# ElesionKyrie/Extreme-Video-Compression-With-Prediction-Using-Pre-trainded-Diffusion-Models-

Measured on AMD Instinct MI355X. Metric: decoded frames/sec (128x128x30) at q3, higher is better.
Workload: dtype f32

## Files before the change

extreme-video-compression-with-prediction-using-pre-trainded-diffusion-models-_amd/csrc/conv_igemm.hip:

```cpp
#include <hip/hip_runtime.h>
#include <stdint.h>
#include <stdio.h>
#include "../../include/evc_hip.h"

typedef float f32x16 __attribute__((ext_vector_type(16)));
typedef __attribute__((address_space(3))) void lds_void;
typedef const __attribute__((address_space(1))) void glb_void;

#ifndef EVC_CONV_TAIL
#define EVC_CONV_TAIL 1
#endif
#ifndef EVC_CONV_TM1
#define EVC_CONV_TM1 1
#endif
#ifndef EVC_SPLIT_WIDE_TILES
#define EVC_SPLIT_WIDE_TILES 1
#endif

#ifndef EVC_SPLIT_INTERLEAVE
#define EVC_SPLIT_INTERLEAVE 5
#endif

namespace {

constexpr int BM_MAX = 128;
constexpr int KC = 16;

constexpr int MODE_PLAIN = 0, MODE_AFFINE = 1, MODE_AFFINE_SILU = 2, MODE_SILU = 3, MODE_RELU = 4;

struct ConvK {
    const float* src0; const float* src1; int C0; int C1; int ld0; int ld1;
    const float* coef_a; const float* coef_s;
    const float* w; const float* bias; const float* res; int ld_res;
    float out_scale; int act_out;
    float* out; int ld_out;
    int B, H, W, Co, CoPad, KH, KW;
    int M, HW, nchunk, nsteps, steps_per_split, splits;
    float* ws;
    float* stats;
    const float* w_hdr;
    const unsigned* in_bound;
    int tail_first, tail_splits, tail_sps, tail_rows;
    int cut_chunk;
    const float* x2_src0; const float* x2_src1; int x2_C0, x2_C1, x2_ld0, x2_ld1;
    const char* x2_w;
    const float* x2_hdr;
    const unsigned* x2_bound;
    int bound_stride, generic_epi;
};

__device__ __forceinline__ float bound_scale(unsigned bits) {
    const float b = sqrtf(__uint_as_float(bits));
    if (!(b < 3.0e38f)) return __builtin_nanf("");
    return b > 0.f ? ldexpf(1.0f, 6 - ilogbf(b)) : 1.0f;
}
__device__ __forceinline__ int bound_index(const ConvK& p, int m) { return p.bound_stride ? min(m, p.M - 1) / p.HW : 0; }
__device__ __forceinline__ float in_scale(const ConvK& p, int m) {
    if (!p.in_bound) return 1.0f;
    return bound_scale(p.in_bound[bound_index(p, m)]);
}

__device__ __forceinline__ float silu_f(float v) { return v * __builtin_amdgcn_rcpf(1.0f + __expf(-v)); }

__device__ __forceinline__ float act_fn(float v, int act) {
    if (act == EVC_ACT_SILU) return silu_f(v);
    if (act == EVC_ACT_RELU) return v < 0.f ? 0.f : v;
    return v;
}

template <int MODE>
__device__ __forceinline__ float4 transform(float4 v, const float4& a, const float4& s, bool ok) {
    if (MODE == MODE_AFFINE || MODE == MODE_AFFINE_SILU) {
        v.x = v.x * a.x + s.x; v.y = v.y * a.y + s.y; v.z = v.z * a.z + s.z; v.w = v.w * a.w + s.w;
    }
    if (MODE == MODE_AFFINE_SILU || MODE == MODE_SILU) {
        v.x = silu_f(v.x); v.y = silu_f(v.y); v.z = silu_f(v.z); v.w = silu_f(v.w);
    }
    if (MODE == MODE_RELU) {
        v.x = v.x < 0.f ? 0.f : v.x; v.y = v.y < 0.f ? 0.f : v.y; v.z = v.z < 0.f ? 0.f : v.z; v.w = v.w < 0.f ? 0.f : v.w;
    }
    v.x = ok ? v.x : 0.f; v.y = ok ? v.y : 0.f; v.z = ok ? v.z : 0.f; v.w = ok ? v.w : 0.f;
    return v;
}

template <int TM, int TN>
__device__ __forceinline__ void mfma_group(f32x16 (&acc)[TM][TN], const float4 (&a)[TM], const float4 (&b)[TN]) {
#define EVC_MFMA_E(e)                                                                                   \
    _Pragma("unroll") for (int i = 0; i < TM; ++i) _Pragma("unroll") for (int j = 0; j < TN; ++j)      \
        acc[i][j] = __builtin_amdgcn_mfma_f32_32x32x2f32(a[i].e, b[j].e, acc[i][j], 0, 0, 0);
    EVC_MFMA_E(x) EVC_MFMA_E(y) EVC_MFMA_E(z) EVC_MFMA_E(w)
#undef EVC_MFMA_E
}

template <int TM, int TN, int WM, bool PARTIAL, bool RES, bool STATS, bool ACT>
__device__ __forceinline__ void conv_epilogue_full(const ConvK& p, f32x16 (&acc)[TM][TN], int m0, int n0, int split,
                                                   int wm, int wn, int l31, int half, bool tail) {
    constexpr int BM = 32 * TM * WM;
    const int ws_m0 = tail ? p.tail_first * BM : 0;
    const size_t ws_M = tail ? (size_t)p.tail_rows : (size_t)p.M;
    const float ascale = p.w_hdr ? p.w_hdr[0] / in_scale(p, m0) : 1.0f;
// ... 966 lines not shown
            __builtin_amdgcn_sched_barrier(0);
            store_a(ab ^ 1);
            __builtin_amdgcn_sched_barrier(0);
            EVC_RR_TERMS(SP::NTERM / 2, SP::NTERM)
            __builtin_amdgcn_sched_barrier(0);
            __syncthreads();
            wb ^= 1; ++sidx;
        }
    }
#undef EVC_RR_TERMS
#undef EVC_RR_FRAGS
#undef EVC_RR_NEXT_W

    conv_epilogue<TM, TN, WM>(p, acc, m0, n0, split, wm, wn, l31, half, tail);
}

template <bool PARTIAL, bool RES, bool STATS, bool ACT>
__device__ __forceinline__ void wide_epilogue_t(const ConvK& p, f32x16 (&acc)[4][3], char* lds, int m0, int n0, int split,
                                                int wave, int lane, bool tail) {
    constexpr int TM = 4, TN = 3, BM = 256, RS = 36;
    const int wm = wave >> 1, wn = wave & 1;
    const int l31 = lane & 31, half = lane >> 5;
    const int ws_m0 = tail ? p.tail_first * BM : 0;
    const size_t ws_M = tail ? (size_t)p.tail_rows : (size_t)p.M;
    const float ascale = p.w_hdr[0] / in_scale(p, m0);
    const float oscale = p.out_scale;
    const bool has_res = RES && (!ACT || p.res != nullptr), has_stats = STATS && (!ACT || p.stats != nullptr);
    float* const patch0 = reinterpret_cast<float*>(lds) + wave * 2 * 32 * RS;
    const int wr = lane >> 3, wc = (lane & 7) * 4;
    const int mw = m0 + wm * 32 * TM;
    const int prow = 4 * half * RS + l31;
    constexpr int RD = 4;
    float4 rq[RD][4];
    const auto res_load = [&](int t, float4 (&dst)[4]) {
        const int jj = t / TM, ii = t - jj * TM;
        const float* rp = p.res + (size_t)(mw + ii * 32 + wr) * p.ld_res + n0 + wn * 32 * TN + jj * 32 + wc;
#pragma unroll
        for (int k = 0; k < 4; ++k) dst[k] = *reinterpret_cast<const float4*>(rp + (size_t)(8 * k) * p.ld_res);
    };
    if (has_res) {
#pragma unroll
        for (int t = 0; t < RD - 1; ++t) res_load(t, rq[t]);
    }
#pragma unroll
    for (int j = 0; j < TN; ++j) {
        const int cj = n0 + wn * 32 * TN + j * 32;
        const float bias = (!PARTIAL && p.bias) ? p.bias[cj + l31] : 0.f;
        float4 ssum = make_float4(0.f, 0.f, 0.f, 0.f), ssq = make_float4(0.f, 0.f, 0.f, 0.f);
#pragma unroll
        for (int i = 0; i < TM; ++i) {
            const int mb = mw + i * 32;
            const int tt = j * TM + i;
            if (has_res && tt + RD - 1 < TM * TN) res_load(tt + RD - 1, rq[(tt + RD - 1) % RD]);
            float* const P = patch0 + ((i * TN + j) & 1) * 32 * RS;
#pragma unroll
            for (int r = 0; r < 16; ++r) P[prow + ((r & 3) + 8 * (r >> 2)) * RS] = acc[i][j][r] * ascale + bias;
#pragma unroll
            for (int k = 0; k < 4; ++k) {
                float4 q = *reinterpret_cast<const float4*>(P + (wr + 8 * k) * RS + wc);
                const int m = mb + wr + 8 * k;
                if (!PARTIAL) {
                    if (has_res) { const float4& rr = rq[tt % RD][k]; q.x += rr.x; q.y += rr.y; q.z += rr.z; q.w += rr.w; }
                    q.x *= oscale; q.y *= oscale; q.z *= oscale; q.w *= oscale;
                    if (ACT) { q.x = act_fn(q.x, p.act_out); q.y = act_fn(q.y, p.act_out); q.z = act_fn(q.z, p.act_out); q.w = act_fn(q.w, p.act_out); }
                    if (STATS) {
                        ssum.x += q.x; ssum.y += q.y; ssum.z += q.z; ssum.w += q.w;
                        ssq.x += q.x * q.x; ssq.y += q.y * q.y; ssq.z += q.z * q.z; ssq.w += q.w * q.w;
                    }
                }
                float* dst = PARTIAL ? p.ws + ((size_t)split * ws_M + (m - ws_m0)) * p.Co + cj + wc
                                     : p.out + (size_t)m * p.ld_out + cj + wc;
                *reinterpret_cast<float4*>(dst) = q;
            }
            if (has_stats && (i & 1)) {
#pragma unroll
                for (int d = 8; d <= 32; d <<= 1) {
                    ssum.x += __shfl_xor(ssum.x, d); ssum.y += __shfl_xor(ssum.y, d); ssum.z += __shfl_xor(ssum.z, d); ssum.w += __shfl_xor(ssum.w, d);
                    ssq.x += __shfl_xor(ssq.x, d); ssq.y += __shfl_xor(ssq.y, d); ssq.z += __shfl_xor(ssq.z, d); ssq.w += __shfl_xor(ssq.w, d);
                }
                if (wr == 0) {
                    float* sp = p.stats + ((size_t)(m0 / 64 + wm * 2 + (i >> 1)) * p.Co + cj + wc) * 2;
                    *reinterpret_cast<float4*>(sp) = make_float4(ssum.x, ssq.x, ssum.y, ssq.y);
                    *reinterpret_cast<float4*>(sp + 4) = make_float4(ssum.z, ssq.z, ssum.w, ssq.w);
                }
                ssum = make_float4(0.f, 0.f, 0.f, 0.f); ssq = make_float4(0.f, 0.f, 0.f, 0.f);
            }
        }
    }
}

__device__ __forceinline__ void wide_epilogue(const ConvK& p, f32x16 (&acc)[4][3], char* lds, int m0, int n0, int split,
                                              int wave, int lane, bool tail) {
    const bool partial = p.splits > 1 || tail;
    if (partial) wide_epilogue_t<true, false, false, false>(p, acc, lds, m0, n0, split, wave, lane, tail);
    else if (p.act_out != EVC_ACT_NONE) wide_epilogue_t<false, true, true, true>(p, acc, lds, m0, n0, split, wave, lane, tail);
    else if (p.res && p.stats) wide_epilogue_t<false, true, true, false>(p, acc, lds, m0, n0, split, wave, lane, tail);
    else if (p.stats) wide_epilogue_t<false, false, true, false>(p, acc, lds, m0, n0, split, wave, lane, tail);
    else if (p.res) wide_epilogue_t<false, true, false, false>(p, acc, lds, m0, n0, split, wave, lane, tail);
    else wide_epilogue_t<false, false, false, false>(p, acc, lds, m0, n0, split, wave, lane, tail);
}

#ifndef EVC_WIDE_VMEM_EVERY
#define EVC_WIDE_VMEM_EVERY 36
#endif
#ifndef EVC_WIDE_BDIST
#define EVC_WIDE_BDIST 1
#endif
#ifndef EVC_WIDE_BUFFER_LOADS
#define EVC_WIDE_BUFFER_LOADS 0
#endif
#ifndef EVC_WIDE_ABL
#define EVC_WIDE_ABL 0
#endif
#ifdef EVC_WIDE_STAMPS
__device__ unsigned long long g_wide_stamps[8192 * 8];
#define EVC_STAMP(k) if (threadIdx.x == 0) g_wide_stamps[(blockIdx.x & 8191) * 8 + (k)] = __builtin_readcyclecounter();
#else
#define EVC_STAMP(k)
#endif
template <int MODE, int NU, bool X2>
__global__ __launch_bounds__(256, 1) void conv_wide_kernel(ConvK p) {
    typedef Split<2> SP;
    typedef f16x8 vec;
    constexpr int TM = 4, TN = 3, BM = 256, BN = 192, RB = 32;
    constexpr bool HAS_COEF = MODE == MODE_AFFINE || MODE == MODE_AFFINE_SILU;
    extern __shared__ __attribute__((aligned(16))) char smem_b[];
    const int W = p.W, SW = W + 2;
    const int R = BM / W;
    const int SPX = (R + 2) * SW;
    const int APL = SPX * RB;
    const int HPL = SPX * 16;
    char* const As = smem_b;

    const int tid = threadIdx.x;
    const int lane = tid & 63;
    const int wave = __builtin_amdgcn_readfirstlane(tid >> 6);
    const int wm = wave >> 1, wn = wave & 1;
    const int l31 = lane & 31, half = lane >> 5;

#ifdef EVC_WIDE_STAGGER_TEST
    if (blockIdx.x < 256) for (int q = 0; q < (int)((blockIdx.x >> 3) & 3) * EVC_WIDE_STAGGER_TEST; ++q) __builtin_amdgcn_s_sleep(127);
#endif
    EVC_STAMP(0)
    const bool tail = (int)blockIdx.x >= p.tail_first;
    const int tq = tail ? ((int)blockIdx.x - p.tail_first) / p.tail_splits : 0;
    const int m0 = (tail ? p.tail_first + tq : (int)blockIdx.x) * BM;
    const int n0 = blockIdx.y * BN;
    const int split = tail ? (int)blockIdx.x - p.tail_first - tq * p.tail_splits : (int)blockIdx.z;
    const int sps = tail ? p.tail_sps : p.steps_per_split;
    const int c_begin = p.cut_chunk ? (split ? p.cut_chunk : 0) : min(p.nchunk, split * (sps / 9));
    const int c_end = p.cut_chunk ? (split ? p.nchunk : p.cut_chunk) : min(p.nchunk, c_begin + sps / 9);

    const int bimg = m0 / p.HW;
    const int y0 = (m0 - bimg * p.HW) / W;
    const int Ct = p.C0 + p.C1;

    const int kh = tid & 1;
    unsigned goff0[NU], goff1[NU];
    int slds[NU];
    bool sval[NU], sex[NU];
#pragma unroll
    for (int k = 0; k < NU; ++k) {
        int pp = (tid + 256 * k) >> 1;
        if (pp >= (R + 2) * W) pp = tid >> 1;
        const int sr = pp / W, x = pp - sr * W;
        sex[k] = true;
        const int y = y0 + sr - 1;
        sval[k] = sex[k] && y >= 0 && y < p.H;
        const unsigned pix = (unsigned)((bimg * p.H + (sval[k] ? y : 0)) * W + x);
        goff0[k] = (pix * (unsigned)p.ld0 + 8u * kh) * 4u;
        goff1[k] = (pix * (unsigned)p.ld1 + 8u * kh) * 4u;
        const int spx = (sex[k] ? sr : 0) * SW + x + 1;
// ... 35 lines not shown
        }
    };
#endif

    const float xscale = F16_ACT_SCALE * in_scale(p, m0);
    float4 xr[NU][2], ca[2], cs[2];
    vec a[TM][2];
    auto stage_load = [&](int k, int c) {
        const int cc = c * KC;
        const bool first = cc < p.C0;
        const char* src = reinterpret_cast<const char*>(first ? p.src0 : p.src1);
        const unsigned o = (first ? goff0[k] : goff1[k]) + (unsigned)(first ? cc : cc - p.C0) * 4u;
        xr[k][0] = *reinterpret_cast<const float4*>(src + o);
        xr[k][1] = *reinterpret_cast<const float4*>(src + o + 16);
    };
    auto coef_load = [&](int c) {
        if (HAS_COEF) {
            const size_t co = (size_t)bimg * Ct + c * KC + 8 * kh;
            ca[0] = *reinterpret_cast<const float4*>(p.coef_a + co);
            ca[1] = *reinterpret_cast<const float4*>(p.coef_a + co + 4);
            cs[0] = *reinterpret_cast<const float4*>(p.coef_s + co);
            cs[1] = *reinterpret_cast<const float4*>(p.coef_s + co + 4);
        }
    };
    auto stage_store = [&](int k, int buf) {
        vec pl[2];
        SP::split(transform<MODE>(xr[k][0], ca[0], cs[0], sval[k]), transform<MODE>(xr[k][1], ca[1], cs[1], sval[k]), xscale, pl);
        char* A = As + buf * 2 * APL + slds[k];
        *reinterpret_cast<vec*>(A) = pl[0];
        *reinterpret_cast<vec*>(A + APL) = pl[1];
    };
    auto read_a = [&](int i, const char* img, int toff) {
        a[i][0] = *reinterpret_cast<const vec*>(img + abase[i] + toff);
        a[i][1] = *reinterpret_cast<const vec*>(img + APL + abase[i] + toff);
    };

    f32x16 acc[TM][TN];
#pragma unroll
    for (int i = 0; i < TM; ++i)
#pragma unroll
        for (int j = 0; j < TN; ++j)
#pragma unroll
            for (int r = 0; r < 16; ++r) acc[i][j][r] = 0.f;

    vec b[3][TN][2];
    const bool early = !X2 && c_begin < c_end;
    if (early) {
        coef_load(c_begin);
#pragma unroll
        for (int k = 0; k < NU; ++k) stage_load(k, c_begin);
        load_b(b[0], c_begin, 0);
    }
    EVC_STAMP(5)
    {
        const int nimg = X2 ? 3 : 2;
        const int per_img = (R + 2) * 2 * 4;
        for (int u = tid; u < nimg * per_img; u += 256) {
            const int img = u / per_img, q = u - img * per_img;
            const int ph = q & 3, side = (q >> 2) & 1, row = q >> 3;
            const int spx = row * SW + (side ? W + 1 : 0);
            *reinterpret_cast<float4*>(As + img * 2 * APL + (ph >> 1) * APL + (ph & 1) * HPL + spx * 16) = make_float4(0.f, 0.f, 0.f, 0.f);
        }
    }
    __syncthreads();

#define EVC_PIN(x) asm volatile("" : "+v"(x))
#define EVC_PIN4(f) asm volatile("" : "+v"((f).x), "+v"((f).y), "+v"((f).z), "+v"((f).w))
#define EVC_WIDE_MFMA_I(I, BB)                                                                          \
    _Pragma("unroll") for (int t_ = 0; t_ < SP::NTERM; ++t_)                                            \
        _Pragma("unroll") for (int j = 0; j < TN; ++j)                                                  \
            acc[I][j] = SP::mfma(a[I][SP::qa(t_)], BB[j][SP::qb(t_)], acc[I][j]);

    if constexpr (X2) {
        const int nch2 = (p.x2_C0 + p.x2_C1) / KC;
        const int nsp = tail ? p.tail_splits : p.splits;
        const int per = (nch2 + nsp - 1) / nsp;
        const int c2b = min(nch2, split * per), c2e = min(nch2, c2b + per);
        float s2 = 1.0f;
        {
            const float bb = sqrtf(__uint_as_float(p.x2_bound[bound_index(p, m0)]));
            if (!(bb < 3.0e38f)) s2 = __builtin_nanf("");
            else if (bb > 0.f) s2 = ldexpf(1.0f, 6 - ilogbf(bb));
        }
        const float xscale2 = F16_ACT_SCALE * s2;
        const unsigned slab2 = 2u * planeB;
        float4 x2r[2][2][2];
        unsigned x2o0[2], x2o1[2];
        int x2l[2];
#pragma unroll
        for (int k = 0; k < 2; ++k) {
            const int pp = (tid + 256 * k) >> 1;
            const int r = pp / W, x = pp - r * W;
            x2o0[k] = ((unsigned)(m0 + pp) * (unsigned)p.x2_ld0 + 8u * kh) * 4u;
            x2o1[k] = ((unsigned)(m0 + pp) * (unsigned)p.x2_ld1 + 8u * kh) * 4u;
            x2l[k] = kh * HPL + ((r + 1) * SW + x + 1) * 16;
        }
        auto load2 = [&](int c, float4 (&xr2)[2][2]) {
            const int cc = c * KC;
            const bool first = cc < p.x2_C0;
            const char* src = reinterpret_cast<const char*>(first ? p.x2_src0 : p.x2_src1);
            const unsigned cb = (unsigned)(first ? cc : cc - p.x2_C0) * 4u;
#pragma unroll
            for (int k = 0; k < 2; ++k) {
                const unsigned o = (first ? x2o0[k] : x2o1[k]) + cb;
                xr2[k][0] = *reinterpret_cast<const float4*>(src + o);
                xr2[k][1] = *reinterpret_cast<const float4*>(src + o + 16);
            }
        };
        auto store2 = [&](int buf, float4 (&xr2)[2][2]) {
            const float4 z = make_float4(0.f, 0.f, 0.f, 0.f);
#pragma unroll
            for (int k = 0; k < 2; ++k) {
                vec pl[2];
                SP::split(transform<MODE_PLAIN>(xr2[k][0], z, z, true), transform<MODE_PLAIN>(xr2[k][1], z, z, true), xscale2, pl);
                char* A = As + buf * 2 * APL + x2l[k];
                *reinterpret_cast<vec*>(A) = pl[0];
                *reinterpret_cast<vec*>(A + APL) = pl[1];
            }
        };
        vec b2[2][TN][2];
        auto load_b2 = [&](vec (&bb)[TN][2], int c) {
            const char* wt = p.x2_w + (unsigned)c * slab2;
#pragma unroll
            for (int j = 0; j < TN; ++j) {
                bb[j][0] = *reinterpret_cast<const vec*>(wt + wlane + j * 32 * RB);
                bb[j][1] = *reinterpret_cast<const vec*>(wt + planeB + wlane + j * 32 * RB);
            }
        };
        const int n2 = c2e - c2b;
        if (n2 > 0) {
            const auto clampc = [&](int c) { return min(c, c2e - 1); };
            load2(c2b, x2r[0]);
            load2(clampc(c2b + 1), x2r[1]);
            load_b2(b2[0], c2b);
            store2(0, x2r[0]);
            store2(1, x2r[1]);
            load2(clampc(c2b + 2), x2r[0]);
            load2(clampc(c2b + 3), x2r[1]);
            __syncthreads();
#pragma unroll
            for (int i = 0; i < TM; ++i) read_a(i, As, tap_off(4));
            int ring = 0;
#define EVC_WIDE_X2_STEP(BCUR, BNXT, XR)                                                                    \
            {                                                                                           \
                const int rn1 = ring == 2 ? 0 : ring + 1, rn2 = rn1 == 2 ? 0 : rn1 + 1;                 \
                _Pragma("unroll") for (int j = 0; j < TN; ++j) { EVC_PIN(BCUR[j][0]); EVC_PIN(BCUR[j][1]); } \
                _Pragma("unroll") for (int k = 0; k < 2; ++k) { EVC_PIN4(XR[k][0]); EVC_PIN4(XR[k][1]); } \
                load_b2(BNXT, clampc(c + 1));                                                           \
                const char* An = As + rn1 * 2 * APL;                                                    \
                _Pragma("unroll") for (int i = 0; i < TM; ++i) {                                        \
                    EVC_PIN(a[i][0]); EVC_PIN(a[i][1]);                                                 \
                    EVC_WIDE_MFMA_I(i, BCUR)                                                            \
                    read_a(i, An, tap_off(4));                                                          \
                }                                                                                       \
                store2(rn2, XR);                                                       \
                _Pragma("unroll") for (int m = 0; m < 36; ++m) {                                        \
                    if (m == 0) __builtin_amdgcn_sched_group_barrier(0x020, 6, 0);                      \
                    __builtin_amdgcn_sched_group_barrier(0x008, 1, 0);                                  \
                    __builtin_amdgcn_sched_group_barrier(0x402, 3, 0);                                  \
                    if (m % 9 == 8) __builtin_amdgcn_sched_group_barrier(0x100, 2, 0);                  \
                }                                                                                       \
                __builtin_amdgcn_sched_group_barrier(0x200, 4, 0);                                      \
                __builtin_amdgcn_sched_barrier(0);                                                      \
                load2(clampc(c + 4), XR);                                \
                asm volatile("s_waitcnt lgkmcnt(0)\n\ts_barrier" ::: "memory");                         \
                __builtin_amdgcn_sched_barrier(0);                                                      \
                ring = rn1;                                                                             \
            }
            int c = c2b;
            for (; c + 1 < c2e; c += 2) {
                EVC_WIDE_X2_STEP(b2[0], b2[1], x2r[0])
                ++c;
                EVC_WIDE_X2_STEP(b2[1], b2[0], x2r[1])
                --c;
            }
            if (c < c2e) EVC_WIDE_X2_STEP(b2[0], b2[1], x2r[0])
#undef EVC_WIDE_X2_STEP
        }
        __syncthreads();
        const float r = (p.x2_hdr[0] / s2) / (p.w_hdr[0] / in_scale(p, m0));
#pragma unroll
        for (int i = 0; i < TM; ++i)
#pragma unroll
            for (int j = 0; j < TN; ++j)
#pragma unroll
                for (int e = 0; e < 16; ++e) acc[i][j][e] *= r;
    }

    EVC_STAMP(6)
    if (c_begin < c_end) {
        if (!early) {
            coef_load(c_begin);
#pragma unroll
            for (int k = 0; k < NU; ++k) stage_load(k, c_begin);
            load_b(b[0], c_begin, 0);
        }
        if (EVC_WIDE_BDIST == 2) load_b(b[1], c_begin, 1);
#pragma unroll
        for (int k = 0; k < NU; ++k) stage_store(k, 0);
        EVC_STAMP(7)
        __syncthreads();
#pragma unroll
        for (int i = 0; i < TM; ++i) read_a(i, As, 0);
    }
    EVC_STAMP(1)
    for (int c = c_begin; c < c_end; ++c) {
        const int ab = (c - c_begin) & 1;
        const int cn = min(c + 1, c_end - 1);
        const char* Acur = As + ab * 2 * APL;
        const char* Anxt = As + (ab ^ 1) * 2 * APL;
#define EVC_WIDE_STEP(T, LOADK, STOREK, TAIL_CODE)                                                      \
        {                                                                                               \
            _Pragma("unroll") for (int j = 0; j < TN; ++j) { EVC_PIN(b[T % 3][j][0]); EVC_PIN(b[T % 3][j][1]); } \
            if constexpr (STOREK >= 0 && STOREK < NU) { EVC_PIN4(xr[STOREK < 0 ? 0 : STOREK][0]); EVC_PIN4(xr[STOREK < 0 ? 0 : STOREK][1]); } \
            if constexpr (STOREK == 0 && HAS_COEF) { EVC_PIN4(ca[0]); EVC_PIN4(ca[1]); EVC_PIN4(cs[0]); EVC_PIN4(cs[1]); } \
            if (EVC_WIDE_ABL & 64) load_b(b[(T + EVC_WIDE_BDIST) % 3], c_begin, 0);    \
            else if (!(EVC_WIDE_ABL & 2)) load_b(b[(T + EVC_WIDE_BDIST) % 3], (T + EVC_WIDE_BDIST < 9) ? c : cn, (T + EVC_WIDE_BDIST) % 9); \
            if (T == 0 && !(EVC_WIDE_ABL & 8)) coef_load(cn);                                           \
            if constexpr (LOADK >= 0 && LOADK < NU && !(EVC_WIDE_ABL & 8)) stage_load(LOADK < 0 ? 0 : LOADK, cn); \
            const char* An = (T == 8) ? Anxt : Acur;                    \
            const int toff = tap_off((T + 1) % 9);                                                      \
            _Pragma("unroll") for (int i = 0; i < TM; ++i) {                                            \
                EVC_PIN(a[i][0]); EVC_PIN(a[i][1]);                                                     \
                EVC_WIDE_MFMA_I(i, b[T % 3])                                                            \
                if (!(EVC_WIDE_ABL & 4)) read_a(i, An, toff);                                           \
            }                                                                                           \
            if constexpr (STOREK >= 0 && STOREK < NU && !(EVC_WIDE_ABL & 1)) stage_store(STOREK < 0 ? 0 : STOREK, ab ^ 1); \
             \
             \
            _Pragma("unroll") for (int m = 0; m < 36; ++m) {                                            \
                if (m % EVC_WIDE_VMEM_EVERY == 0) __builtin_amdgcn_sched_group_barrier(0x020, 1, 0);    \
                __builtin_amdgcn_sched_group_barrier(0x008, 1, 0);                                      \
                __builtin_amdgcn_sched_group_barrier(0x402, 4, 0);                                      \
                if (m % 9 == 8) __builtin_amdgcn_sched_group_barrier(0x100, 2, 0);                      \
            }                                                                                           \
            __builtin_amdgcn_sched_group_barrier(0x200, 2, 0);                                          \
            __builtin_amdgcn_sched_barrier(0);                                                          \
            TAIL_CODE                                                                                   \
            __builtin_amdgcn_sched_barrier(0);                                                          \
        }
        EVC_WIDE_STEP(0, 0, -1, )
        EVC_WIDE_STEP(1, 1, -1, )
        EVC_WIDE_STEP(2, 2, 0, )
        EVC_WIDE_STEP(3, 3, 1, )
        EVC_WIDE_STEP(4, -1, 2, )
        EVC_WIDE_STEP(5, -1, 3, )
        EVC_WIDE_STEP(6, -1, -1, )
        EVC_WIDE_STEP(7, -1, -1, asm volatile("s_waitcnt lgkmcnt(0)\n\ts_barrier" ::: "memory");)
// ... 191 lines not shown
    }
}

extern "C" int evc_conv_pack_weights(const float* w, void* packed, int Co, int Ci, int KH, int KW, int arith,
                                     void* stream) {
    if (arith == EVC_ARITH_F32) return evc_conv_pack_weights_f32(w, (float*)packed, Co, Ci, KH, KW, stream);
    if (arith != EVC_ARITH_BF16X6 && arith != EVC_ARITH_F16X3) return EVC_EINVAL;
    if (!w || !packed || Co <= 0 || Ci <= 0 || Ci % KC != 0 || KH <= 0 || KW <= 0) return EVC_EINVAL;
    const long long total = evc_conv_packed_floats(Co, Ci, KH, KW);
    int grid = (int)((total + 255) / 256 > 4096 ? 4096 : (total + 255) / 256);
    hipStream_t st = (hipStream_t)stream;
    if (arith == EVC_ARITH_BF16X6) {
        hipLaunchKernelGGL(conv_pack_split_kernel, dim3(grid), dim3(256), 0, st, w, (__bf16*)packed, Co,
                           evc_conv_co_pad(Co), Ci, KH, KW);
    } else {
        if (hipMemsetAsync(packed, 0, F16_HDR_BYTES, st) != hipSuccess) return EVC_ELAUNCH;
        const size_t n = (size_t)Co * Ci * KH * KW;
        hipLaunchKernelGGL(conv_absmax_kernel, dim3(grid), dim3(256), 0, st, w, n, reinterpret_cast<unsigned*>(packed) + 2);
        hipLaunchKernelGGL(conv_pack_f16_kernel, dim3(grid), dim3(256), 0, st, w, (char*)packed, Co,
                           evc_conv_co_pad(Co), Ci, KH, KW);
    }
    return hipGetLastError() == hipSuccess ? EVC_OK : EVC_ELAUNCH;
}

static int conv_validate(const evc_conv_args* a) {
    if (!a || !a->src0 || !a->w_packed || !a->out) return EVC_EINVAL;
    if (a->C0 <= 0 || a->C0 % KC != 0 || a->C1 < 0 || a->C1 % KC != 0) return EVC_EINVAL;
    if (a->C1 > 0 && !a->src1) return EVC_EINVAL;
    if ((a->ld0 != 0 && (a->ld0 < a->C0 || (a->ld0 & 3))) || (a->ld1 != 0 && (a->ld1 < a->C1 || (a->ld1 & 3))))
        return EVC_EINVAL;
    if ((a->coef_a == nullptr) != (a->coef_s == nullptr)) return EVC_EINVAL;
    if (a->B <= 0 || a->H <= 0 || a->W <= 0 || a->Co <= 0) return EVC_EINVAL;
    if (a->KH <= 0 || a->KW <= 0 || !(a->KH & 1) || !(a->KW & 1)) return EVC_EINVAL;
    if (a->ld_out < a->Co || (a->res && a->ld_res < a->Co)) return EVC_EINVAL;
    if ((long long)a->B * a->H * a->W > 0x7fffffffLL) return EVC_EINVAL;
    if (a->arith != EVC_ARITH_F32 && a->arith != EVC_ARITH_BF16X6 && a->arith != EVC_ARITH_F16X3) return EVC_EINVAL;
    if (a->x2_w_packed) {
        if (!a->x2_src0 || !a->x2_bound || a->x2_C0 <= 0 || a->x2_C0 % KC != 0 || a->x2_C1 < 0 || a->x2_C1 % KC != 0) return EVC_EINVAL;
        if (a->x2_C1 > 0 && !a->x2_src1) return EVC_EINVAL;
        if ((a->x2_ld0 != 0 && (a->x2_ld0 < a->x2_C0 || (a->x2_ld0 & 3))) || (a->x2_ld1 != 0 && (a->x2_ld1 < a->x2_C1 || (a->x2_ld1 & 3))))
            return EVC_EINVAL;
    }
    return EVC_OK;
}

struct TileCfg { int tm, tn, bm, bn; long long tiles; int splits; int reuse; int wide; int steps_per_split;
                 int tail_first, tail_tiles, tail_splits, tail_sps;
                 int cut_chunk; };
static int g_wide_cut = 1;
static int g_tail_split = EVC_CONV_TAIL;
static int g_wide_tiles = EVC_SPLIT_WIDE_TILES;
static int g_no_reuse = 0;
static int g_wide_mid = 1;
static int g_wide256 = 1;
static int g_force_tm = 0;

static void split_tile_cfg(const evc_conv_args* a, long long M, long long ntile, int nsteps, TileCfg& c, bool rr_ok, bool inv) {
    const double K = (double)a->KH * a->KW * (a->C0 + a->C1);
    const bool f16 = a->arith == EVC_ARITH_F16X3 && rr_ok;
    const double E = f16 ? 20.0 : 6.0, F2 = f16 ? 1.5 : 1.0;
    const auto grid_time = [&](long long n, double sps) {
        const long long R = n / 512, rem = n - R * 512;
        return (sps + E) * ((double)R * F2 + (rem == 0 ? 0.0 : (rem <= 256 && f16 ? 1.0 : F2)));
    };
    double best = 1e300;
    int best_tm = 2, best_s = 1;
    c.tail_first = 0; c.tail_tiles = 0; c.tail_splits = 1; c.tail_sps = 0;
    for (int tm = 2; tm >= 1; --tm) {
        if (!inv && g_force_tm && tm != g_force_tm) continue;
        const long long tiles = ((M + 64 * tm - 1) / (64 * tm)) * ntile;
        const int smax = a->splits > 0 ? a->splits : (nsteps / 4 < 1 ? 1 : (nsteps / 4 > 32 ? 32 : nsteps / 4));
        for (int s = a->splits > 0 ? a->splits : 1; s <= smax; ++s) {
            const double sps = (double)((nsteps + s - 1) / s);
            const double slab_mb = (double)s * (double)M * a->Co * 4.0 / 1e6;
            const double pen = s > 1 ? 1.0 + (slab_mb > 192.0 ? 300.0 : 40.0) * s / K : 1.0;
            const double tmf = tm == 1 ? (a->KH * a->KW > 1 ? 0.5 / (rr_ok ? 0.55 : 0.75) : 0.5) : 1.0;
            const double t = grid_time(tiles * s, sps) * pen * tmf;
            if (t < best * 0.9999) { best = t; best_tm = tm; best_s = s; }
        }
    }
    c.tm = best_tm;
    c.bm = 64 * c.tm;
    c.tiles = ((M + c.bm - 1) / c.bm) * ntile;
    c.splits = best_s;
    if (!inv && rr_ok && g_tail_split && a->splits <= 0 && !g_force_tm && M % 128 == 0) {
        const long long tm_all = M / 128, wgs = tm_all * ntile;
        const long long R = wgs / 512;
        const long long main_m = R * 512 / ntile, tail_m = tm_all - main_m;
        const int unit = 3 * 9;
        if (R >= 1 && tail_m > 0 && nsteps >= 2 * unit) {
            int ts = (int)(512 / (tail_m * ntile));
            if (ts > nsteps / unit) ts = nsteps / unit;
            if (ts >= 2) {
                int sps = (nsteps + ts - 1) / ts;
                sps = (sps + 2) / 3 * 3;
                ts = (nsteps + sps - 1) / sps;
                const double t_tail = grid_time(main_m * ntile, (double)nsteps) +
                                      grid_time(tail_m * ntile * ts, (double)sps) * (1.0 + 40.0 * ts / K);
                if (ts >= 2 && t_tail < best * 0.98) {
                    c.tm = 2; c.bm = 128; c.tiles = wgs; c.splits = 1;
                    c.tail_first = (int)main_m; c.tail_tiles = (int)tail_m; c.tail_splits = ts; c.tail_sps = sps;
                }
            }
        }
    }
}

static inline bool is_split_arith(int arith) { return arith == EVC_ARITH_BF16X6 || arith == EVC_ARITH_F16X3; }
static inline int arith_planes(int arith) { return arith == EVC_ARITH_F16X3 ? 2 : 3; }
constexpr long long LDS_CAP = 160 * 1024;

static long long rr_lds_bytes(int np, int bm, int W, int bn) {
    return (long long)np * 32 * (2LL * (bm / W) * (W + 2) + 2LL * bn);
}

static long long wide_lds_bytes(int W, bool x2) { return (x2 ? 6LL : 4LL) * (256 / W + 2) * (W + 2) * 32; }

static bool wide_ok(const evc_conv_args* a, bool inv) {
    const bool mode_ok = a->coef_a ? a->act_in == EVC_ACT_SILU : a->act_in == EVC_ACT_NONE;
    return (inv || g_wide256) && mode_ok && a->arith == EVC_ARITH_F16X3 && a->KH == 3 && a->KW == 3 && a->Co % 192 == 0 &&
           (a->W == 16 || a->W == 32 || a->W == 64 || a->W == 128) && ((long long)a->H * a->W) % 256 == 0 &&
           a->ld_out % 4 == 0 && (!a->res || a->ld_res % 4 == 0);
}

static TileCfg conv_tile_cfg_at(const evc_conv_args* a, bool inv) {
    TileCfg c;
    c.wide = 0;
    c.cut_chunk = 0;
    const long long M = (long long)a->B * a->H * a->W;
    const int CoPad = evc_conv_co_pad(a->Co);
    c.tn = pick_tn(CoPad);
    c.bn = 64 * c.tn;
    const long long ntile = CoPad / c.bn;
    const int nsteps = a->KH * a->KW * ((a->C0 + a->C1) / KC);
    c.reuse = 0;
    if (is_split_arith(a->arith)) {
        const int np = arith_planes(a->arith);
        const bool rr_ok = (inv || !g_no_reuse) && a->KH == 3 && a->KW == 3 && a->W >= 4 && 128 % a->W == 0 &&
                           rr_lds_bytes(np, 128, a->W, c.bn) <= LDS_CAP;
        split_tile_cfg(a, M, ntile, nsteps, c, rr_ok, inv);
        if (rr_ok && c.tm == 2) c.reuse = 1;
        if (!inv && c.reuse && c.splits == 1 && !c.tail_tiles && g_wide_tiles && M % 256 == 0 && rr_lds_bytes(np, 256, a->W, c.bn) <= LDS_CAP) {
            const long long t256 = (M / 256) * ntile;
            if ((t256 >= 512 && t256 % 256 == 0) || t256 >= 6 * 256) {
                c.bm = 256;
                c.tiles = t256;
            }
        }
    } else {
        c.tail_first = 0; c.tail_tiles = 0; c.tail_splits = 1; c.tail_sps = 0;
        c.tm = (!EVC_CONV_TM1 || ((M + 127) / 128) * ntile >= 64) ? 2 : 1;
        if (g_force_tm && !inv) c.tm = g_force_tm;
        c.bm = 64 * c.tm;
        c.tiles = ((M + c.bm - 1) / c.bm) * ntile;
        long long splits = 1;
        if (a->splits > 0) splits = a->splits;
        else if (c.tiles < 384) {
            splits = (640 + c.tiles / 2) / c.tiles;
            const int max_by_steps = nsteps / 8 > 0 ? nsteps / 8 : 1;
            if (splits > max_by_steps) splits = max_by_steps;
            if (splits > 32) splits = 32;
            if (splits < 1) splits = 1;
        }
        c.splits = (int)splits;
    }
    if (wide_ok(a, inv) && a->splits <= 0 && (inv || !g_force_tm)) {
        const long long tm_all = M / 256, nt = a->Co / 192, wgs = tm_all * nt;
        if (wgs >= 256) {
            const int nchunk = (a->C0 + a->C1) / KC;
// ... 26 lines not shown
            if (best_s > 0 && wgs * best_s >= 128) {
                const int cps = (nchunk + best_s - 1) / best_s;
                c.wide = 1; c.reuse = 0; c.tm = 4; c.tn = 3; c.bm = 256; c.bn = 192; c.tiles = wgs;
                c.tail_first = 0; c.tail_tiles = 0; c.tail_splits = 1; c.tail_sps = 0;
                c.splits = (nchunk + cps - 1) / cps;
                c.steps_per_split = cps * 9;
                if ((inv || g_wide_cut) && best_s == 1 && wgs > 128 && nchunk >= 6) {
                    const long long idle = 256 - wgs, r = (wgs + idle - 1) / idle;
                    const double slab_mb = 2.0 * M * a->Co * 4.0 / 1e6;
                    const double comb = 2.0 * 2000.0 * (5.0 + slab_mb / 4.0);
                    int cut = 0;
                    double t_cut = best_t * 0.95;
                    for (int sh = 1; sh <= nchunk / 2; ++sh) {
                        const double tl = 23000.0 + 13900.0 * (nchunk - sh), ts = (double)r * (23000.0 + 13900.0 * sh);
                        const double t = (tl > ts ? tl : ts) + comb;
                        if (t < t_cut) { t_cut = t; cut = nchunk - sh; }
                    }
                    if (cut > 0) { c.splits = 2; c.cut_chunk = cut; c.steps_per_split = cut * 9; }
                }
                return c;
            }
        }
    }
    const int unit = c.reuse ? a->KW : 1;
    int sps = (nsteps + c.splits - 1) / c.splits;
    sps = (sps + unit - 1) / unit * unit;
    c.steps_per_split = sps;
    c.splits = (nsteps + sps - 1) / sps;
    return c;
}

#define EVC_INVARIANT_PLAN_REVISION 1
static TileCfg conv_tile_cfg(const evc_conv_args* a) {
    if (!a->invariant) return conv_tile_cfg_at(a, false);
    evc_conv_args r = *a;
    r.B = EVC_INVARIANT_REF_BATCH;
    TileCfg c = conv_tile_cfg_at(&r, true);
    const long long M = (long long)a->B * a->H * a->W;
    c.tiles = ((M + c.bm - 1) / c.bm) * (evc_conv_co_pad(a->Co) / c.bn);
    return c;
}

extern "C" int evc_invariant_plan_revision(void) { return EVC_INVARIANT_PLAN_REVISION; }

extern "C" int evc_conv_set_option(const char* name, int value) {
    if (!name) return EVC_EINVAL;
    const auto is = [&](const char* s) { int i = 0; while (s[i] && s[i] == name[i]) ++i; return s[i] == 0 && name[i] == 0; };
    if (is("wide_tiles")) { g_wide_tiles = value; return EVC_OK; }
    if (is("row_reuse")) { g_no_reuse = !value; return EVC_OK; }
    if (is("tail_split")) { g_tail_split = value; return EVC_OK; }
    if (is("wide256")) { g_wide256 = value; return EVC_OK; }
    if (is("wide_mid")) { g_wide_mid = value; return EVC_OK; }
    if (is("wide_cut")) { g_wide_cut = value; return EVC_OK; }
    return EVC_EINVAL;
}

extern "C" int evc_conv_fused_1x1_supported(const evc_conv_args* a) {
    if (conv_validate(a) != EVC_OK) return 0;
    if (a->arith != EVC_ARITH_F16X3 || a->KH != 3 || a->KW != 3) return 0;
    const TileCfg c = conv_tile_cfg(a);
    if (a->invariant && ((long long)a->H * a->W) % c.bm != 0) return 0;
    return (c.reuse == 1 || c.wide) ? 1 : 0;
}

extern "C" int evc_conv_kernel_name(const evc_conv_args* a, char* buf, int n) {
    if (!buf || n <= 0 || conv_validate(a) != EVC_OK) return EVC_EINVAL;
    int mode;
    if (a->coef_a) mode = a->act_in == EVC_ACT_SILU ? MODE_AFFINE_SILU : MODE_AFFINE;
    else mode = a->act_in == EVC_ACT_SILU ? MODE_SILU : a->act_in == EVC_ACT_RELU ? MODE_RELU : MODE_PLAIN;
    const TileCfg c = conv_tile_cfg(a);
    int len;
    if (c.wide) len = snprintf(buf, n, "conv_wide_kernel<%d, %d, %s>", mode, a->W == 128 ? 4 : 3, a->x2_w_packed ? "true" : "false");
    else if (is_split_arith(a->arith)) {
        const int np = arith_planes(a->arith);
        if (c.reuse) len = snprintf(buf, n, "conv_split_rr_kernel<%d, %d, %d, %d>", np, c.bm == 256 ? 4 : 2, c.tn, mode);
        else if (np == 3) len = snprintf(buf, n, "conv_split_kernel<%d, %d, %d>", c.tm, c.tn, mode);
        else len = snprintf(buf, n, "conv_splitn_kernel<2, %d, %d, %d>", c.tm, c.tn, mode);
    } else len = snprintf(buf, n, "conv_igemm_kernel<%d, %d, %d>", c.tm, c.tn, mode);
    return len;
}

extern "C" int evc_conv_choose_splits(const evc_conv_args* a) {
    if (conv_validate(a) != EVC_OK) return EVC_EINVAL;
    return conv_tile_cfg(a).splits;
}

extern "C" int evc_conv_stats_splits(const evc_conv_args* a) {
    if (conv_validate(a) != EVC_OK) return 0;
    const int HW = a->H * a->W;
    if (HW % 64 != 0) return 0;
    const TileCfg c = conv_tile_cfg(a);
    if (c.splits > 1 || c.wide) return HW / 64;
    if (a->invariant && HW % c.bm != 0) return 0;
    const long long M = (long long)a->B * HW;
    const int CoPad = evc_conv_co_pad(a->Co);
    if (M % c.bm != 0 || a->Co != CoPad || a->Co % c.bn != 0) return 0;
    return HW / (32 * c.tm);
}

extern "C" int evc_conv_plan_query(const evc_conv_args* a, evc_conv_plan* out) {
    if (!out || conv_validate(a) != EVC_OK) return EVC_EINVAL;
    const TileCfg c = conv_tile_cfg(a);
    if (evc_conv_kernel_name(a, out->kernel, (int)sizeof(out->kernel)) < 0) return EVC_EINVAL;
    out->tile_m = c.bm; out->tile_n = c.bn; out->splits = c.splits; out->steps_per_split = c.steps_per_split;
    out->cut_chunk = c.wide ? c.cut_chunk : 0;
    out->tail_tiles = c.tail_tiles; out->tail_splits = c.tail_tiles ? c.tail_splits : 1;
// ... 117 lines not shown
    if (rc != EVC_OK) return rc;
    int mode;
    if (a->coef_a) {
        if (a->act_in == EVC_ACT_SILU) mode = MODE_AFFINE_SILU;
        else if (a->act_in == EVC_ACT_NONE) mode = MODE_AFFINE;
        else return EVC_EUNSUPPORTED;
    } else {
        mode = a->act_in == EVC_ACT_SILU ? MODE_SILU : a->act_in == EVC_ACT_RELU ? MODE_RELU : MODE_PLAIN;
        if (a->act_in != EVC_ACT_NONE && a->act_in != EVC_ACT_SILU && a->act_in != EVC_ACT_RELU) return EVC_EINVAL;
    }
    ConvK k;
    k.src0 = a->src0; k.src1 = a->src1 ? a->src1 : a->src0; k.C0 = a->C0; k.C1 = a->C1;
    k.ld0 = a->ld0 > 0 ? a->ld0 : a->C0; k.ld1 = a->ld1 > 0 ? a->ld1 : (a->C1 > 0 ? a->C1 : k.ld0);
    k.coef_a = a->coef_a; k.coef_s = a->coef_s;
    k.w = a->w_packed; k.bias = a->bias; k.res = a->res; k.ld_res = a->ld_res;
    k.w_hdr = nullptr;
    k.in_bound = nullptr;
    if (a->in_bound) {
        if (a->arith != EVC_ARITH_F16X3) return EVC_EINVAL;
        k.in_bound = a->in_bound;
    }
    if (a->arith == EVC_ARITH_F16X3) {
        k.w_hdr = a->w_packed;
        k.w = reinterpret_cast<const float*>(reinterpret_cast<const char*>(a->w_packed) + F16_HDR_BYTES);
    }
    k.out_scale = a->out_scale; k.act_out = a->act_out; k.out = a->out; k.ld_out = a->ld_out;
    k.B = a->B; k.H = a->H; k.W = a->W; k.Co = a->Co; k.CoPad = evc_conv_co_pad(a->Co);
    k.KH = a->KH; k.KW = a->KW;
    k.M = a->B * a->H * a->W; k.HW = a->H * a->W;
    if ((long long)k.M * k.ld0 * 4 >= (1LL << 32) || (long long)k.M * k.ld1 * 4 >= (1LL << 32)) return EVC_EUNSUPPORTED;
    if (a->KH * a->KW > 32) return EVC_EUNSUPPORTED;
    k.nchunk = (a->C0 + a->C1) / KC;
    k.nsteps = a->KH * a->KW * k.nchunk;
    const TileCfg cfg = conv_tile_cfg(a);
    k.splits = cfg.splits;
    k.steps_per_split = cfg.steps_per_split;
    k.ws = ws;
    if ((k.splits > 1 || cfg.tail_tiles) && !ws) return EVC_EINVAL;
    k.stats = k.splits > 1 ? nullptr : a->stats_out;
    if (a->stats_out && evc_conv_stats_splits(a) == 0) return EVC_EINVAL;
    k.x2_w = nullptr; k.x2_hdr = nullptr; k.x2_bound = nullptr; k.x2_src0 = k.x2_src1 = nullptr;
    k.x2_C0 = k.x2_C1 = k.x2_ld0 = k.x2_ld1 = 0;
    if (a->x2_w_packed) {
        if (a->arith != EVC_ARITH_F16X3 || a->KH != 3 || a->KW != 3 || !(cfg.reuse == 1 || cfg.wide)) return EVC_EUNSUPPORTED;
        k.x2_src0 = a->x2_src0; k.x2_src1 = a->x2_src1 ? a->x2_src1 : a->x2_src0;
        k.x2_C0 = a->x2_C0; k.x2_C1 = a->x2_C1;
        k.x2_ld0 = a->x2_ld0 > 0 ? a->x2_ld0 : a->x2_C0;
        k.x2_ld1 = a->x2_ld1 > 0 ? a->x2_ld1 : (a->x2_C1 > 0 ? a->x2_C1 : k.x2_ld0);
        if ((long long)k.M * k.x2_ld0 * 4 >= (1LL << 32) || (long long)k.M * k.x2_ld1 * 4 >= (1LL << 32)) return EVC_EUNSUPPORTED;
        k.x2_hdr = a->x2_w_packed;
        k.x2_w = reinterpret_cast<const char*>(a->x2_w_packed) + F16_HDR_BYTES;
        k.x2_bound = a->x2_bound;
    }
    k.bound_stride = 0; k.generic_epi = 0;
    if (a->invariant) {
        const bool whole = k.HW % cfg.bm == 0;
        k.bound_stride = 1;
        k.generic_epi = whole ? 0 : 1;
        if (!whole && (cfg.reuse || cfg.wide) && (a->in_bound || a->x2_w_packed)) return EVC_EUNSUPPORTED;
    }
    k.tail_first = 0x7fffffff; k.tail_splits = 1; k.tail_sps = 0; k.tail_rows = 0;
    k.cut_chunk = cfg.wide ? cfg.cut_chunk : 0;
    if (cfg.tail_tiles) {
        k.tail_first = cfg.tail_first; k.tail_splits = cfg.tail_splits; k.tail_sps = cfg.tail_sps;
        k.tail_rows = cfg.tail_tiles * cfg.bm;
    }

    dim3 grid((k.M + cfg.bm - 1) / cfg.bm, k.CoPad / cfg.bn, k.splits);
    if (cfg.tail_tiles) grid.x = cfg.tail_first + cfg.tail_tiles * cfg.tail_splits;
    hipStream_t st = (hipStream_t)stream;
    if (ev_start && hipEventRecord(ev_start, st) != hipSuccess) return EVC_ELAUNCH;
    if (cfg.wide) {
        rc = launch_wide(mode, a->W == 128 ? 4 : 3, a->x2_w_packed != nullptr, grid, (size_t)wide_lds_bytes(a->W, a->x2_w_packed != nullptr), st, k);
    } else if (is_split_arith(a->arith)) {
        const int np = arith_planes(a->arith);
        if (cfg.reuse) {
            const size_t lds_rr = (size_t)rr_lds_bytes(np, cfg.bm, a->W, cfg.bn);
#define EVC_RR4_3(TN) launch_split_rr<3, 4, TN>(mode, grid, lds_rr, st, k)
#define EVC_RR2_3(TN) launch_split_rr<3, 2, TN>(mode, grid, lds_rr, st, k)
#define EVC_RR4_2(TN) launch_split_rr<2, 4, TN>(mode, grid, lds_rr, st, k)
#define EVC_RR2_2(TN) launch_split_rr<2, 2, TN>(mode, grid, lds_rr, st, k)
            if (np == 3) rc = cfg.bm == 256 ? EVC_TN_SWITCH(cfg.tn, EVC_RR4_3) : EVC_TN_SWITCH(cfg.tn, EVC_RR2_3);
            else rc = cfg.bm == 256 ? EVC_TN_SWITCH(cfg.tn, EVC_RR4_2) : EVC_TN_SWITCH(cfg.tn, EVC_RR2_2);
#undef EVC_RR4_3
#undef EVC_RR2_3
#undef EVC_RR4_2
#undef EVC_RR2_2
        } else {
            const size_t lds = (size_t)2 * np * (cfg.bm + cfg.bn) * 32;
#define EVC_S3_2(TN) launch_split3<2, TN>(mode, grid, lds, st, k)
#define EVC_S3_1(TN) launch_split3<1, TN>(mode, grid, lds, st, k)
#define EVC_S2_2(TN) launch_split2<2, TN>(mode, grid, lds, st, k)
#define EVC_S2_1(TN) launch_split2<1, TN>(mode, grid, lds, st, k)
            if (np == 3) rc = cfg.tm == 2 ? EVC_TN_SWITCH(cfg.tn, EVC_S3_2) : EVC_TN_SWITCH(cfg.tn, EVC_S3_1);
            else rc = cfg.tm == 2 ? EVC_TN_SWITCH(cfg.tn, EVC_S2_2) : EVC_TN_SWITCH(cfg.tn, EVC_S2_1);
#undef EVC_S3_2
#undef EVC_S3_1
#undef EVC_S2_2
#undef EVC_S2_1
        }
    } else {
        const size_t lds = (size_t)2 * (cfg.bm + cfg.bn) * KC * sizeof(float);
#define EVC_F_2(TN) launch_mode<2, TN>(mode, grid, lds, st, k)
#define EVC_F_1(TN) launch_mode<1, TN>(mode, grid, lds, st, k)
        rc = cfg.tm == 2 ? EVC_TN_SWITCH(cfg.tn, EVC_F_2) : EVC_TN_SWITCH(cfg.tn, EVC_F_1);
#undef EVC_F_2
#undef EVC_F_1
    }
    if (rc != EVC_OK) return rc;
    if (hipGetLastError() != hipSuccess) return EVC_ELAUNCH;
    if (ev_conv_end && hipEventRecord(ev_conv_end, st) != hipSuccess) return EVC_ELAUNCH;
    if (k.splits > 1) {
        hipLaunchKernelGGL(conv_splitk_reduce_kernel, dim3((k.M + 63) / 64, (k.Co + 63) / 64), dim3(1024), 0, st, ws,
                           k.splits, k.M, k.Co, a->bias, a->res, a->ld_res, a->out_scale, a->act_out, a->out,
                           a->ld_out, a->stats_out);
        if (hipGetLastError() != hipSuccess) return EVC_ELAUNCH;
    }
    if (cfg.tail_tiles) {
        const size_t m0 = (size_t)cfg.tail_first * cfg.bm;
        hipLaunchKernelGGL(conv_splitk_reduce_kernel, dim3((k.tail_rows + 63) / 64, (k.Co + 63) / 64), dim3(1024), 0, st, ws,
                           k.tail_splits, k.tail_rows, k.Co, a->bias, a->res ? a->res + m0 * a->ld_res : nullptr, a->ld_res,
                           a->out_scale, a->act_out, a->out + m0 * a->ld_out, a->ld_out,
                           a->stats_out ? a->stats_out + (m0 / 64) * k.Co * 2 : nullptr);
        if (hipGetLastError() != hipSuccess) return EVC_ELAUNCH;
    }
    return EVC_OK;
// ... 2 lines not shown
```

Before: 36.73.

## Add grouped multi-buffer ring pipeline for wide-conv X2 (1x1 shortcut) phase

Adds a new path for the secondary X2 input in the wide conv kernel. It stages several channel chunks into an LDS ring buffer and only synchronizes every G steps, instead of once per chunk. Loads, splits and stores are interleaved with MFMAs using sched_group_barrier hints. The aim is to cut per-chunk barriers and expose more load latency hiding, at the cost of more LDS for the ring and more register pressure. Halo zeroing is deferred until after the X2 phase, since the ring overwrites that LDS.

New measurement: 36.91 (median of 6 runs). About the same (+0.5%).

```diff
diff --git a/extreme-video-compression-with-prediction-using-pre-trainded-diffusion-models-_amd/csrc/conv_igemm.hip b/extreme-video-compression-with-prediction-using-pre-trainded-diffusion-models-_amd/csrc/conv_igemm.hip
--- a/extreme-video-compression-with-prediction-using-pre-trainded-diffusion-models-_amd/csrc/conv_igemm.hip
+++ b/extreme-video-compression-with-prediction-using-pre-trainded-diffusion-models-_amd/csrc/conv_igemm.hip
@@ -46,6 +46,7 @@
     const char* x2_w;
     const float* x2_hdr;
     const unsigned* x2_bound;
+    int x2_group;
     int bound_stride, generic_epi;
 };
 
@@ -1118,7 +1119,7 @@
             const int mb = mw + i * 32;
             const int tt = j * TM + i;
             if (has_res && tt + RD - 1 < TM * TN) res_load(tt + RD - 1, rq[(tt + RD - 1) % RD]);
-            float* const P = patch0 + ((i * TN + j) & 1) * 32 * RS;
+            float* const P = patch0 + (tt & 1) * 32 * RS;
 #pragma unroll
             for (int r = 0; r < 16; ++r) P[prow + ((r & 3) + 8 * (r >> 2)) * RS] = acc[i][j][r] * ascale + bias;
 #pragma unroll
@@ -1184,6 +1185,7 @@
 #else
 #define EVC_STAMP(k)
 #endif
+template <int N> struct WideIntC { static constexpr int value = N; };
 template <int MODE, int NU, bool X2>
 __global__ __launch_bounds__(256, 1) void conv_wide_kernel(ConvK p) {
     typedef Split<2> SP;
@@ -1325,8 +1327,7 @@
         load_b(b[0], c_begin, 0);
     }
     EVC_STAMP(5)
-    {
-        const int nimg = X2 ? 3 : 2;
+    const auto zero_halo = [&](int nimg) {
         const int per_img = (R + 2) * 2 * 4;
         for (int u = tid; u < nimg * per_img; u += 256) {
             const int img = u / per_img, q = u - img * per_img;
@@ -1334,7 +1335,9 @@
             const int spx = row * SW + (side ? W + 1 : 0);
             *reinterpret_cast<float4*>(As + img * 2 * APL + (ph >> 1) * APL + (ph & 1) * HPL + spx * 16) = make_float4(0.f, 0.f, 0.f, 0.f);
         }
-    }
+    };
+    const bool x2g = X2 && p.x2_group > 1;
+    if (!x2g) zero_halo(X2 ? 3 : 2);
     __syncthreads();
 
 #define EVC_PIN(x) asm volatile("" : "+v"(x))
@@ -1401,7 +1404,86 @@
             }
         };
         const int n2 = c2e - c2b;
-        if (n2 > 0) {
+        const auto x2_grouped = [&](auto gtag) __attribute__((always_inline)) {
+            constexpr int G = decltype(gtag)::value, D = G + 1, NR = 2 * G;
+            constexpr int HS2 = 256 * 16 + 128, PL2 = 2 * HS2, IMG2 = 2 * PL2;
+            float4 xg[4][2][2], xt[2][2];
+            int lo2[2];
+#pragma unroll
+            for (int k = 0; k < 2; ++k) lo2[k] = kh * HS2 + ((tid + 256 * k) >> 1) * 16;
+            const int a2 = half * HS2 + (wm * 128 + l31) * 16;
+            const auto store2g = [&](char* img, float4 (&xr2)[2][2]) {
+                const float4 z = make_float4(0.f, 0.f, 0.f, 0.f);
+#pragma unroll
+                for (int k = 0; k < 2; ++k) {
+                    vec pl[2];
+                    SP::split(transform<MODE_PLAIN>(xr2[k][0], z, z, true), transform<MODE_PLAIN>(xr2[k][1], z, z, true), xscale2, pl);
+                    *reinterpret_cast<vec*>(img + lo2[k]) = pl[0];
+                    *reinterpret_cast<vec*>(img + PL2 + lo2[k]) = pl[1];
+                }
+            };
+            const auto read_a2 = [&](int i, const char* img) {
+                a[i][0] = *reinterpret_cast<const vec*>(img + a2 + i * 512);
+                a[i][1] = *reinterpret_cast<const vec*>(img + PL2 + a2 + i * 512);
+            };
+            const auto clampc = [&](int c) { return min(c, c2e - 1); };
+            vec bg[4][TN][2];
+#pragma unroll
+            for (int q = 0; q < 4; ++q) load2(clampc(c2b + q), xg[q]);
+            if constexpr (D > 4) load2(clampc(c2b + 4), xt);
+#pragma unroll
+            for (int q = 0; q < 3; ++q) load_b2(bg[q], clampc(c2b + q));
+#pragma unroll
+            for (int q = 0; q < (D < 4 ? D : 4); ++q) store2g(As + q * IMG2, xg[q]);
+            if constexpr (D > 4) store2g(As + 4 * IMG2, xt);
+#pragma unroll
+            for (int q = (D < 4 ? 4 : D); q < D + 4; ++q) load2(clampc(c2b + q), xg[q % 4]);
+            __syncthreads();
+#pragma unroll
+            for (int i = 0; i < TM; ++i) read_a2(i, As);
+            int rs = IMG2, ws = D * IMG2;
+#define EVC_WIDE_X2G_STEP(K, LIVE)                                                                      \
+            {                                                                                           \
+                constexpr int SET = (K + D) % 4;                                                        \
+                _Pragma("unroll") for (int j = 0; j < TN; ++j) { EVC_PIN(bg[K][j][0]); EVC_PIN(bg[K][j][1]); } \
+                if constexpr (LIVE) { _Pragma("unroll") for (int k = 0; k < 2; ++k) { EVC_PIN4(xg[SET][k][0]); EVC_PIN4(xg[SET][k][1]); } } \
+                load_b2(bg[(K + 3) % 4], clampc(c + K + 3));                                            \
+                const char* An = As + rs;                                                               \
+                _Pragma("unroll") for (int i = 0; i < TM; ++i) {                                        \
+                    EVC_PIN(a[i][0]); EVC_PIN(a[i][1]);                                                 \
+                    EVC_WIDE_MFMA_I(i, bg[K])                                                           \
+                    read_a2(i, An);                                                                     \
+                }                                                                                       \
+                if constexpr (LIVE) store2g(As + ws, xg[SET]);                 \
+                _Pragma("unroll") for (int m = 0; m < 36; ++m) {                                        \
+                    if (m == 0) __builtin_amdgcn_sched_group_barrier(0x020, 6, 0);                      \
+                    __builtin_amdgcn_sched_group_barrier(0x008, 1, 0);                                  \
+                    __builtin_amdgcn_sched_group_barrier(0x402, LIVE ? 6 : 1, 0);                       \
+                    if (m % 9 == 8) __builtin_amdgcn_sched_group_barrier(0x100, 2, 0);                  \
+                }                                                                                       \
+                if constexpr (LIVE) __builtin_amdgcn_sched_group_barrier(0x200, 4, 0);                  \
+                __builtin_amdgcn_sched_barrier(0);                                                      \
+                if constexpr (LIVE) load2(clampc(c + K + D + 4), xg[SET]);    \
+                if constexpr ((K + 2) % G == 0) asm volatile("s_waitcnt lgkmcnt(0)\n\ts_barrier" ::: "memory"); \
+                __builtin_amdgcn_sched_barrier(0);                                                      \
+                rs = rs == (NR - 1) * IMG2 ? 0 : rs + IMG2;                                             \
+                ws = ws == (NR - 1) * IMG2 ? 0 : ws + IMG2;                                             \
+            }
+            int c = c2b;
+            for (; c + 4 <= c2e; c += 4) {
+                EVC_WIDE_X2G_STEP(0, true)
+                EVC_WIDE_X2G_STEP(1, true)
+                EVC_WIDE_X2G_STEP(2, true)
+                EVC_WIDE_X2G_STEP(3, true)
+            }
+            const int rem = c2e - c;
+            if (rem > 0) EVC_WIDE_X2G_STEP(0, false)
+            if (rem > 1) EVC_WIDE_X2G_STEP(1, false)
+            if (rem > 2) EVC_WIDE_X2G_STEP(2, false)
+#undef EVC_WIDE_X2G_STEP
+        };
+        if (n2 > 0 && p.x2_group > 1) x2_grouped(WideIntC<4>{});
+        else if (n2 > 0) {
             const auto clampc = [&](int c) { return min(c, c2e - 1); };
             load2(c2b, x2r[0]);
             load2(clampc(c2b + 1), x2r[1]);
@@ -1467,6 +1549,9 @@
 #pragma unroll
             for (int k = 0; k < NU; ++k) stage_load(k, c_begin);
             load_b(b[0], c_begin, 0);
+        }
+        if constexpr (X2) {
+            if (x2g) zero_halo(2);
         }
         if (EVC_WIDE_BDIST == 2) load_b(b[1], c_begin, 1);
 #pragma unroll
@@ -1764,6 +1849,7 @@
 static int g_wide_tiles = EVC_SPLIT_WIDE_TILES;
 static int g_no_reuse = 0;
 static int g_wide_mid = 1;
+static int g_wide_x2_group = 4;
 static int g_wide256 = 1;
 static int g_force_tm = 0;
 
@@ -1826,7 +1912,13 @@
     return (long long)np * 32 * (2LL * (bm / W) * (W + 2) + 2LL * bn);
 }
 
-static long long wide_lds_bytes(int W, bool x2) { return (x2 ? 6LL : 4LL) * (256 / W + 2) * (W + 2) * 32; }
+static long long wide_lds_bytes(int W, bool x2, int x2_group) {
+    const long long img = 2LL * (256 / W + 2) * (W + 2) * 32;
+    if (!x2) return 2 * img;
+    if (x2_group <= 1) return 3 * img;
+    const long long ring = 2LL * x2_group * 4 * (256 * 16 + 128);
+    return ring > 2 * img ? ring : 2 * img;
+}
 
 static bool wide_ok(const evc_conv_args* a, bool inv) {
     const bool mode_ok = a->coef_a ? a->act_in == EVC_ACT_SILU : a->act_in == EVC_ACT_NONE;
@@ -1959,6 +2051,11 @@
     if (is("wide256")) { g_wide256 = value; return EVC_OK; }
     if (is("wide_mid")) { g_wide_mid = value; return EVC_OK; }
     if (is("wide_cut")) { g_wide_cut = value; return EVC_OK; }
+    if (is("wide_x2_group")) {
+        if (value != 1 && value != 4) return EVC_EINVAL;
+        g_wide_x2_group = value;
+        return EVC_OK;
+    }
     return EVC_EINVAL;
 }
 
@@ -2182,6 +2279,7 @@
         k.x2_w = reinterpret_cast<const char*>(a->x2_w_packed) + F16_HDR_BYTES;
         k.x2_bound = a->x2_bound;
     }
+    k.x2_group = g_wide_x2_group;
     k.bound_stride = 0; k.generic_epi = 0;
     if (a->invariant) {
         const bool whole = k.HW % cfg.bm == 0;
@@ -2201,7 +2299,7 @@
     hipStream_t st = (hipStream_t)stream;
     if (ev_start && hipEventRecord(ev_start, st) != hipSuccess) return EVC_ELAUNCH;
     if (cfg.wide) {
-        rc = launch_wide(mode, a->W == 128 ? 4 : 3, a->x2_w_packed != nullptr, grid, (size_t)wide_lds_bytes(a->W, a->x2_w_packed != nullptr), st, k);
+        rc = launch_wide(mode, a->W == 128 ? 4 : 3, a->x2_w_packed != nullptr, grid, (size_t)wide_lds_bytes(a->W, a->x2_w_packed != nullptr, k.x2_group), st, k);
     } else if (is_split_arith(a->arith)) {
         const int np = arith_planes(a->arith);
         if (cfg.reuse) {
```
